# UBC-AWP/vision-sam3-yolo-lameless

Hardware: AMD Instinct MI355X
Metric: frames/sec (whole node) for YOLO+SAM3+DINOv3 feature extraction, 1080p clips (higher is better)
Workload: dtype f16; 1 GPU; BASELINE cfg#5, dense schedule: fused per-frame path on a synthetic 5 s @ 30 fps 1080p clip (150 unique BGR frames resident in HBM): YOLOv8-l detect (letterbox 384x640, NMS, scale_boxes; f16 plan) -> SAM (Hiera-B+ image encoder + FPN at 1024x1024, box-prompted mask decoder, 1080p mask + statistics + contour features) + DINOv3 ViT-L/16 embed (224x224) on EVERY frame; per-frame records packed, gathe; parallelism=one clip per GPU, 1 GPU(s), one gather per step, streams=7

## Files before the change

### vision-sam3-yolo-lameless_amd/csrc/common.h

```cpp
#pragma once
#include <hip/hip_runtime.h>
#include <stdint.h>
#include <stdio.h>
#include <stdarg.h>
#include "../../include/lmx.h"

typedef _Float16 half_t;
typedef _Float16 half2_t __attribute__((ext_vector_type(2)));
typedef _Float16 half4_t __attribute__((ext_vector_type(4)));
typedef _Float16 half8_t __attribute__((ext_vector_type(8)));
typedef float f32x4 __attribute__((ext_vector_type(4)));
typedef float f32x16 __attribute__((ext_vector_type(16)));
typedef unsigned int u32x4 __attribute__((ext_vector_type(4)));
typedef unsigned int u32x2 __attribute__((ext_vector_type(2)));

void lmx_set_error(const char* fmt, ...);

#define LMX_REQUIRE(cond, ...)            \
  do {                                    \
    if (!(cond)) {                        \
      lmx_set_error(__VA_ARGS__);         \
      return LMX_EINVAL;                  \
    }                                     \
  } while (0)

#define LMX_HIP(call)                                                                   \
  do {                                                                                  \
    hipError_t e_ = (call);                                                             \
    if (e_ != hipSuccess) {                                                             \
      lmx_set_error("%s failed: %s (%s:%d)", #call, hipGetErrorString(e_), __FILE__, __LINE__); \
      return LMX_EHIP;                                                                  \
    }                                                                                   \
  } while (0)

#define LMX_TRY(call)               \
  do {                              \
    const int rc_ = (call);         \
    if (rc_ != LMX_OK) return rc_;  \
  } while (0)

int lmx_stream_device(hipStream_t st, int* dev);
int lmx_cu_count(int dev);
int lmx_persistent_grid(int64_t need, int dev, unsigned* grid);
int lmx_allow_lds(const void* kernel, int bytes, int dev);
int lmx_env_int(const char* name, int dflt);
int lmx_env_set(const char* name);
int lmx_env_char(const char* name);

struct GemmRoute {
  bool dma;
  int BM, BN, BK, NSTAGE, STAG;
  bool rowln = false;
};
#define LMX_ROUTE_NAME(name, cap, ...)                                                                          \
  do {                                                                                                          \
    LMX_REQUIRE((name) != nullptr && (cap) > 0, "%s: no room for the name", __func__);                          \
    LMX_REQUIRE(snprintf((name), (size_t)(cap), __VA_ARGS__) < (cap), "%s: name buffer of %d bytes is too short", __func__, (cap)); \
  } while (0)

static inline int lmx_launch_check(const char* what) {
  hipError_t e = hipGetLastError();
  if (e != hipSuccess) {
    lmx_set_error("launch of %s failed: %s", what, hipGetErrorString(e));
    return LMX_EHIP;
  }
  return LMX_OK;
}

typedef float f32x2 __attribute__((ext_vector_type(2)));

__device__ __forceinline__ f32x2 gelu_pk(f32x2 v) {
  f32x2 vc;
  vc[0] = __builtin_amdgcn_fmed3f(v[0], -4.5f, 4.5f);
  vc[1] = __builtin_amdgcn_fmed3f(v[1], -4.5f, 4.5f);
  const f32x2 u = vc * vc;
  f32x2 p = {-1.223331157e-12f, -1.223331157e-12f};
  p = p * u + 1.524351007e-10f;
  p = p * u + -8.481037793e-09f;
  p = p * u + 2.798429583e-07f;
  p = p * u + -6.151207192e-06f;
  p = p * u + 9.615961466e-05f;
  p = p * u + -1.114801972e-03f;
  p = p * u + 9.814679350e-03f;
  p = p * u + -6.632144717e-02f;
  p = p * u + 3.988863025e-01f;
  const f32x2 g = vc * p;
  return v * g + 0.5f * v;
}
__device__ __forceinline__ float gelu_1(float v) {
  const f32x2 r = gelu_pk(f32x2{v, v});
  return r[0];
}

__device__ __forceinline__ float lmx_act(float v, int act) {
  if (act == LMX_ACT_SILU) return v * __builtin_amdgcn_rcpf(1.0f + __builtin_amdgcn_exp2f(-v * 1.44269504088896340736f));
  if (act == LMX_ACT_GELU) return gelu_1(v);
  if (act == LMX_ACT_RELU) return fmaxf(v, 0.0f);
  return v;
}

typedef __attribute__((address_space(3))) void* lds_ptr_t;

__device__ __forceinline__ void lds_dma16(__amdgpu_buffer_rsrc_t rs, char* dst_lds, unsigned voffset, int soffset) {
  __builtin_amdgcn_raw_ptr_buffer_load_lds(rs, (lds_ptr_t)dst_lds, 16, voffset, soffset, 0, 0);
}

#define LMX_WAIT_CASE(n) \
  if constexpr (N == n) asm volatile("s_waitcnt vmcnt(" #n ")" ::: "memory")
template <int N>
__device__ __forceinline__ void wait_vmcnt() {
  static_assert(N == 0 || N == 1 || N == 2 || N == 3 || N == 4 || N == 6 || N == 8 || N == 9 || N == 12 || N == 16 || N == 18 || N == 24 ||
                    N == 32,
                "add the literal for this count");
  LMX_WAIT_CASE(0);
  LMX_WAIT_CASE(1);
  LMX_WAIT_CASE(2);
  LMX_WAIT_CASE(3);
  LMX_WAIT_CASE(4);
  LMX_WAIT_CASE(6);
  LMX_WAIT_CASE(8);
  LMX_WAIT_CASE(9);
  LMX_WAIT_CASE(12);
  LMX_WAIT_CASE(16);
  LMX_WAIT_CASE(18);
  LMX_WAIT_CASE(24);
  LMX_WAIT_CASE(32);
}
#undef LMX_WAIT_CASE
template <int PT>
__device__ __forceinline__ void wait_tiles(int y) {
  if (y >= 4)
    wait_vmcnt<4 * PT>();
  else if (y == 3)
    wait_vmcnt<3 * PT>();
  else if (y == 2)
    wait_vmcnt<2 * PT>();
  else if (y == 1)
    wait_vmcnt<PT>();
  else
    wait_vmcnt<0>();
}

static inline bool aligned16(const void* p) { return (((uintptr_t)p) & 15) == 0; }

__device__ __forceinline__ float wave_sum(float v) {
#pragma unroll
  for (int o = 32; o > 0; o >>= 1) v += __shfl_xor(v, o, 64);
  return v;
}
__device__ __forceinline__ float wave_max(float v) {
#pragma unroll
  for (int o = 32; o > 0; o >>= 1) v = fmaxf(v, __shfl_xor(v, o, 64));
  return v;
}

__device__ __forceinline__ float act_exact(float v, int act) {
  if (act == LMX_ACT_SILU) return v / (1.0f + expf(-v));
  if (act == LMX_ACT_RELU) return fmaxf(v, 0.0f);
  if (act == LMX_ACT_GELU) return 0.5f * v * (1.0f + erff(v * 0.70710678118654752440f));
  return v;
}

__device__ __forceinline__ void bil_idx(float scale, int dst, int in_size, int& i0, int& i1, float& l1) {
  float src = scale * ((float)dst + 0.5f) - 0.5f;
  src = src < 0.f ? 0.f : src;
  i0 = (int)src;
  i1 = i0 + (i0 < in_size - 1 ? 1 : 0);
  l1 = src - (float)i0;
}

__device__ __forceinline__ float sample_mid(const float* __restrict__ lg, int L, int T, float sLT, int Y, int X) {
  int y0, y1, x0, x1;
  float ly, lx;
  bil_idx(sLT, Y, L, y0, y1, ly);
  bil_idx(sLT, X, L, x0, x1, lx);
  const float t0 = (1.f - lx) * lg[y0 * L + x0] + lx * lg[y0 * L + x1];
  const float t1 = (1.f - lx) * lg[y1 * L + x0] + lx * lg[y1 * L + x1];
  return (1.f - ly) * t0 + ly * t1;
}
```

### vision-sam3-yolo-lameless_amd/csrc/gemm.hip

```cpp
#include "common.h"
#include <stdlib.h>

namespace {

constexpr int BK = 64;

template <int BM, int BN, int AMODE, int OUT_DT>
__global__ __launch_bounds__(256, 2) void gemm_kernel(const lmx_gemm_desc p) {
  extern __shared__ __attribute__((aligned(16))) char smem[];
  half_t* As = reinterpret_cast<half_t*>(smem);
  half_t* Ws = As + 2 * BM * BK;
  constexpr int FM = BM / 32;
  constexpr int FN = BN / 32;
  constexpr int AI = BM / 32;
  constexpr int WI = BN / 32;

  const int tid = threadIdx.x;
  const int lane = tid & 63;
  const int wave = tid >> 6;
  const int wm = wave & 1, wn = wave >> 1;

  const int nwg = gridDim.x;
  const int bid = blockIdx.x;
  const int q = nwg >> 3, r = nwg & 7, xcd = bid & 7;
// ... 64 lines not shown
#pragma unroll
    for (int i = 0; i < WI; ++i)
      w_st[i] = (w_ok[i] && k_ok) ? *reinterpret_cast<const half8_t*>(W + w_off[i] + k) : zero8;
  };
  auto store_tile = [&](int buf) {
    half_t* as = As + buf * BM * BK;
    half_t* ws = Ws + buf * BN * BK;
#pragma unroll
    for (int i = 0; i < AI; ++i) {
      const int row = r0 + 32 * i;
      *reinterpret_cast<half8_t*>(as + row * BK + ((c ^ (row & 7)) << 3)) = a_st[i];
    }
#pragma unroll
    for (int i = 0; i < WI; ++i) {
      const int row = r0 + 32 * i;
      *reinterpret_cast<half8_t*>(ws + row * BK + ((c ^ (row & 7)) << 3)) = w_st[i];
    }
  };

  f32x4 acc[FM][FN];
#pragma unroll
  for (int i = 0; i < FM; ++i)
#pragma unroll
    for (int j = 0; j < FN; ++j) acc[i][j] = f32x4{0.f, 0.f, 0.f, 0.f};

  const int nk = (p.K + BK - 1) / BK;
  load_tile(0);
  store_tile(0);
  __syncthreads();

  const int frow = lane & 15;
  const int fq = lane >> 4;
  for (int kt = 0; kt < nk; ++kt) {
    const int buf = kt & 1;
    if (kt + 1 < nk) load_tile(kt + 1);
    const half_t* as = As + buf * BM * BK + (wm * (BM / 2) + frow) * BK;
    const half_t* ws = Ws + buf * BN * BK + (wn * (BN / 2) + frow) * BK;
#pragma unroll
    for (int ks = 0; ks < 2; ++ks) {
      const int coff = (((ks << 2) + fq) ^ (frow & 7)) << 3;
      half8_t af[FM], wf[FN];
#pragma unroll
      for (int i = 0; i < FM; ++i) af[i] = *reinterpret_cast<const half8_t*>(as + i * 16 * BK + coff);
#pragma unroll
      for (int j = 0; j < FN; ++j) wf[j] = *reinterpret_cast<const half8_t*>(ws + j * 16 * BK + coff);
#pragma unroll
      for (int i = 0; i < FM; ++i)
#pragma unroll
        for (int j = 0; j < FN; ++j)
          acc[i][j] = __builtin_amdgcn_mfma_f32_16x16x32_f16(wf[j], af[i], acc[i][j], 0, 0, 0);
    }
    if (kt + 1 < nk) store_tile(buf ^ 1);
    __syncthreads();
  }

  if (p.act == LMX_ACT_SWIGLU) {
    if constexpr (OUT_DT == LMX_F16 && FN % 2 == 0) {
      half_t* C = reinterpret_cast<half_t*>(p.C);
#pragma unroll
      for (int i = 0; i < FM; ++i) {
        const int m = m0 + wm * (BM / 2) + i * 16 + frow;
        if (m >= p.M) continue;
#pragma unroll
        for (int j = 0; j < FN; j += 2) {
          const int n = n0 + wn * (BN / 2) + j * 16 + fq * 4;
          if (n >= p.N) continue;
          f32x4 g = acc[i][j], u = acc[i][j + 1];
          if (p.bias) {
            g += *reinterpret_cast<const f32x4*>(p.bias + n);
            u += *reinterpret_cast<const f32x4*>(p.bias + n + 16);
          }
          const int no = (n >> 5) * 16 + (n & 15);
          f32x4 v;
#pragma unroll
          for (int e = 0; e < 4; ++e) v[e] = __fmul_rn(lmx_act(g[e], LMX_ACT_SILU), u[e]);
          if (p.scale) {
            const f32x4 s = *reinterpret_cast<const f32x4*>(p.scale + no);
#pragma unroll
            for (int e = 0; e < 4; ++e) v[e] = __fmul_rn(v[e], s[e]);
          }
          half4_t o;
#pragma unroll
          for (int e = 0; e < 4; ++e) o[e] = (half_t)v[e];
          *reinterpret_cast<half4_t*>(C + (int64_t)m * p.ldc + no) = o;
        }
      }
    }
    return;
  }

#pragma unroll
  for (int i = 0; i < FM; ++i) {
    const int m = m0 + wm * (BM / 2) + i * 16 + frow;
    if (m >= p.M) continue;
    const int mr = p.res_rows > 0 ? m % p.res_rows : m;
#pragma unroll
    for (int j = 0; j < FN; ++j) {
      const int n = n0 + wn * (BN / 2) + j * 16 + fq * 4;
      if (n >= p.N) continue;
      f32x4 v = acc[i][j];
      if (p.bias) {
        const f32x4 b = *reinterpret_cast<const f32x4*>(p.bias + n);
        v += b;
      }
      if (p.act != LMX_ACT_NONE) {
#pragma unroll
        for (int e = 0; e < 4; ++e) v[e] = lmx_act(v[e], p.act);
      }
      if (p.scale) {
        const f32x4 s = *reinterpret_cast<const f32x4*>(p.scale + n);
#pragma unroll
        for (int e = 0; e < 4; ++e) v[e] = __fmul_rn(v[e], s[e]);
      }
      if (OUT_DT == LMX_F32) {
        float* C = reinterpret_cast<float*>(p.C);
        if (p.res) {
          const f32x4 rr = *reinterpret_cast<const f32x4*>(reinterpret_cast<const float*>(p.res) + (int64_t)mr * p.ldr + n);
#pragma unroll
          for (int e = 0; e < 4; ++e) v[e] = __fadd_rn(v[e], rr[e]);
        }
        *reinterpret_cast<f32x4*>(C + (int64_t)m * p.ldc + n) = v;
      } else {
        half_t* C = reinterpret_cast<half_t*>(p.C);
        if (p.res) {
          const half4_t rr =
              *reinterpret_cast<const half4_t*>(reinterpret_cast<const half_t*>(p.res) + (int64_t)mr * p.ldr + n);
#pragma unroll
          for (int e = 0; e < 4; ++e) v[e] = __fadd_rn((float)(half_t)v[e], (float)rr[e]);
        }
        half4_t o;
#pragma unroll
        for (int e = 0; e < 4; ++e) o[e] = (half_t)v[e];
        *reinterpret_cast<half4_t*>(C + (int64_t)m * p.ldc + n) = o;
      }
    }
  }
}

template <int BM, int BN, int AMODE, int OUT_DT>
int launch(const lmx_gemm_desc& d, hipStream_t st) {
  const int MT = (d.M + BM - 1) / BM, NT = (d.N + BN - 1) / BN;
  const size_t smem = (size_t)2 * (BM + BN) * BK * sizeof(half_t);
  int dev;
  LMX_TRY(lmx_stream_device(st, &dev));
  LMX_TRY(lmx_allow_lds(reinterpret_cast<const void*>(&gemm_kernel<BM, BN, AMODE, OUT_DT>), (int)smem, dev));
  hipLaunchKernelGGL((gemm_kernel<BM, BN, AMODE, OUT_DT>), dim3(MT * NT), dim3(256), smem, st, d);
  return lmx_launch_check("gemm_kernel");
}

}

GemmRoute lmx_gemm2_tiling(const lmx_gemm_desc& d);
int lmx_gemm2_launch(const lmx_gemm_desc& d, const GemmRoute& r, hipStream_t st);

static bool dma_ok(const lmx_gemm_desc& d, int m_min, int n_min) {
  const bool a_ok = d.a_mode != 1 || (d.Cin % 32 == 0 && d.H < 32768 && d.W_ < 32768);
  return a_ok && d.M >= m_min && d.N >= n_min && d.N % 8 == 0 && d.ldc % 8 == 0 && aligned16(d.C) &&
         (!d.res || (d.ldr % 8 == 0 && aligned16(d.res)));
}

static int gemm_route(const lmx_gemm_desc* dp, GemmRoute& r) {
  LMX_REQUIRE(dp != nullptr, "lmx_k_gemm: null descriptor");
  const lmx_gemm_desc& d = *dp;
  LMX_REQUIRE(d.A && d.W && d.C, "lmx_k_gemm: null A/W/C");
  LMX_REQUIRE(d.M > 0 && d.N > 0 && d.K > 0, "lmx_k_gemm: empty problem M=%d N=%d K=%d", d.M, d.N, d.K);
  LMX_REQUIRE(d.K % 8 == 0, "lmx_k_gemm: K=%d must be a multiple of 8", d.K);
  LMX_REQUIRE(d.N % 4 == 0, "lmx_k_gemm: N=%d must be a multiple of 4", d.N);
  LMX_REQUIRE(d.lda % 8 == 0, "lmx_k_gemm: lda=%lld must be a multiple of 8", (long long)d.lda);
  const bool gated = d.act == LMX_ACT_SWIGLU;
  LMX_REQUIRE(d.ldc % 4 == 0 && d.ldc >= (gated ? d.N / 2 : d.N), "lmx_k_gemm: bad ldc=%lld", (long long)d.ldc);
  LMX_REQUIRE(aligned16(d.A) && aligned16(d.W), "lmx_k_gemm: A/W must be 16-byte aligned");
  LMX_REQUIRE((((uintptr_t)d.C) & 7) == 0, "lmx_k_gemm: C must be 8-byte aligned");
  LMX_REQUIRE(d.out_dtype == LMX_F16 || d.out_dtype == LMX_F32, "lmx_k_gemm: bad out_dtype %d", d.out_dtype);
  LMX_REQUIRE(d.out_dtype == LMX_F16 || aligned16(d.C), "lmx_k_gemm: f32 C must be 16-byte aligned");
  LMX_REQUIRE(d.act >= LMX_ACT_NONE && d.act <= LMX_ACT_SWIGLU, "lmx_k_gemm: bad act %d", d.act);
  if (gated) {
    LMX_REQUIRE(d.N % 32 == 0, "lmx_k_gemm: LMX_ACT_SWIGLU: N=%d (gate + up rows, interleaved by 16) must be a multiple of 32", d.N);
    LMX_REQUIRE(!d.res, "lmx_k_gemm: LMX_ACT_SWIGLU takes no residual");
    LMX_REQUIRE(d.a_mode == 0 && d.a_rep <= 1 && d.split_k <= 1, "lmx_k_gemm: LMX_ACT_SWIGLU: dense A only (a_mode 0; no pooled rows, convolution, a_rep or split_k); a_mode=%d", d.a_mode);
    LMX_REQUIRE(d.out_dtype == LMX_F16, "lmx_k_gemm: LMX_ACT_SWIGLU writes f16 (one rounding of the f32 product)");
  }
  if (d.bias) LMX_REQUIRE(aligned16(d.bias), "lmx_k_gemm: bias must be 16-byte aligned");
  if (d.scale) LMX_REQUIRE(aligned16(d.scale), "lmx_k_gemm: scale must be 16-byte aligned");
  if (d.res) LMX_REQUIRE(d.ldr % 4 == 0 && d.ldr >= d.N, "lmx_k_gemm: bad ldr=%lld", (long long)d.ldr);
  LMX_REQUIRE(d.res_rows >= 0, "lmx_k_gemm: res_rows");
  if (d.a_mode == 0) {
    LMX_REQUIRE(d.a_rep > 1 || d.lda >= d.K, "lmx_k_gemm: lda=%lld < K=%d", (long long)d.lda, d.K);
  } else if (d.a_mode == 1) {
    LMX_REQUIRE(d.Cin > 0 && d.Cin % 8 == 0, "lmx_k_gemm: conv Cin=%d must be a multiple of 8", d.Cin);
    LMX_REQUIRE(d.K == 9 * d.Cin, "lmx_k_gemm: conv K=%d != 9*Cin=%d", d.K, 9 * d.Cin);
    LMX_REQUIRE(d.conv_stride == 1 || d.conv_stride == 2, "lmx_k_gemm: conv stride %d", d.conv_stride);
    LMX_REQUIRE(d.H > 0 && d.W_ > 0, "lmx_k_gemm: conv H/W");
    LMX_REQUIRE(d.Ho == (d.H + 2 - 3) / d.conv_stride + 1 && d.Wo == (d.W_ + 2 - 3) / d.conv_stride + 1,
                "lmx_k_gemm: conv Ho/Wo (%d,%d) inconsistent with H/W (%d,%d) stride %d", d.Ho, d.Wo, d.H, d.W_,
                d.conv_stride);
    LMX_REQUIRE(d.M % (d.Ho * d.Wo) == 0, "lmx_k_gemm: conv M=%d not a multiple of Ho*Wo", d.M);
    LMX_REQUIRE(d.lda >= d.Cin, "lmx_k_gemm: conv pixel stride lda=%lld < Cin=%d", (long long)d.lda, d.Cin);
  } else if (d.a_mode == 2) {
    LMX_REQUIRE(d.lda >= d.K, "lmx_k_gemm: lda=%lld < K=%d", (long long)d.lda, d.K);
    LMX_REQUIRE(d.H > 0 && d.W_ > 0 && d.H % 2 == 0 && d.W_ % 2 == 0 && d.M % (d.H * d.W_) == 0,
                "lmx_k_gemm: pooled rows need an even H x W token grid that divides M (H=%d W=%d M=%d)", d.H, d.W_, d.M);
    LMX_REQUIRE(!d.res && !d.scale && d.act == LMX_ACT_NONE, "lmx_k_gemm: pooled rows: no residual / scale / activation");
    LMX_REQUIRE(((int64_t)d.M * d.lda + d.K) * 2 < 0x7fffffffll, "lmx_k_gemm: pooled rows: A must be smaller than 2 GB");
    LMX_REQUIRE(dma_ok(d, 512, 96),
                "lmx_k_gemm: pooled rows are built for the LDS-DMA kernel (M >= 512, N >= 96, N %% 8 == 0): use GEMM + maxpool2 for M=%d N=%d", d.M, d.N);
  } else {
    LMX_REQUIRE(false, "lmx_k_gemm: bad a_mode %d", d.a_mode);
  }
  LMX_REQUIRE(d.a_rep >= 0 && d.a_rep <= 3, "lmx_k_gemm: a_rep=%d (0..3)", d.a_rep);
  LMX_REQUIRE(d.split_k >= 0 && d.split_k <= 64, "lmx_k_gemm: split_k=%d (0..64)", d.split_k);
  static const int v1 = lmx_env_char("LMX_GEMM_V1") == '1';
  static const int n64 = lmx_env_char("LMX_GEMM_N64") != '0';
  if (d.ln_out) {
    LMX_REQUIRE(d.out_dtype == LMX_F32 && d.res && d.res_rows == 0, "lmx_k_gemm: ln_out needs f32 output with a full residual (out_dtype=%d res_rows=%d)", d.out_dtype, d.res_rows);
    LMX_REQUIRE(d.N <= 448 && d.N % 16 == 0 && d.K <= 448, "lmx_k_gemm: ln_out: a tile holds whole rows of N <= 448 (N %% 16 == 0) over K <= 448; N=%d K=%d", d.N, d.K);
    LMX_REQUIRE(d.a_mode == 0 && d.a_rep <= 1 && d.split_k <= 1, "lmx_k_gemm: ln_out: dense A only (a_mode=%d a_rep=%d split_k=%d)", d.a_mode, d.a_rep, d.split_k);
    LMX_REQUIRE(d.act == LMX_ACT_NONE && !d.scale, "lmx_k_gemm: ln_out takes no activation and no scale");
    LMX_REQUIRE(d.ln_gamma && d.ln_beta && aligned16(d.ln_gamma) && aligned16(d.ln_beta), "lmx_k_gemm: ln_gamma / ln_beta must be given, 16-byte aligned");
    LMX_REQUIRE(d.ld_ln % 4 == 0 && d.ld_ln >= d.N && (((uintptr_t)d.ln_out) & 7) == 0, "lmx_k_gemm: ln_out must be 8-byte aligned with ld_ln=%lld a multiple of 4, >= N", (long long)d.ld_ln);
    LMX_REQUIRE(aligned16(d.res), "lmx_k_gemm: ln_out: the residual must be 16-byte aligned");
    r = GemmRoute{true, 128, 448, BK, 2, 0, true};
    return LMX_OK;
  }
  bool dma;
  if (d.split_k > 1) {
    LMX_REQUIRE(d.out_dtype == LMX_F32 && d.act == LMX_ACT_NONE && d.a_mode != 2 && d.a_rep <= 1, "lmx_k_gemm: split_k needs f32 output, no activation, a_mode 0 or 1");
    LMX_REQUIRE(d.split_stride >= (int64_t)(d.M - 1) * d.ldc + d.N && d.split_stride % 4 == 0, "lmx_k_gemm: split_stride=%lld", (long long)d.split_stride);
    LMX_REQUIRE((d.K + 63) / 64 >= d.split_k, "lmx_k_gemm: split_k=%d exceeds the k-tiles of K=%d", d.split_k, d.K);
    LMX_REQUIRE(dma_ok(d, 1, 64),
                "lmx_k_gemm: split_k is built into the LDS-DMA kernel only (N >= 64, N %% 8 == 0; conv: Cin %% 32 == 0); M=%d N=%d", d.M, d.N);
    dma = true;
  } else if (d.a_rep > 1) {
    LMX_REQUIRE(d.a_mode == 0 && d.K % d.a_rep == 0 && (d.K / d.a_rep) % 64 == 0, "lmx_k_gemm: a_rep=%d needs a_mode 0 and K / a_rep a multiple of 64 (K=%d)", d.a_rep, d.K);
    LMX_REQUIRE(d.lda >= d.K / d.a_rep, "lmx_k_gemm: lda=%lld < K / a_rep", (long long)d.lda);
    LMX_REQUIRE(dma_ok(d, 512, 96),
                "lmx_k_gemm: a_rep is built into the LDS-DMA kernel only (M >= 512, N >= 96, N %% 8 == 0); M=%d N=%d", d.M, d.N);
    dma = true;
  } else if (d.a_mode == 2) {
    dma = true;
  } else {
    dma = !v1 && dma_ok(d, 512, d.a_mode == 1 && n64 && d.M >= 65536 ? 64 : 96);
  }
  if (dma) {
    r = lmx_gemm2_tiling(d);
  } else {
    const bool narrow = d.N <= 64 || (d.N < 128 && d.N % 128 != 0);
    r = GemmRoute{false, 128, narrow ? 64 : 128, BK, 2, 0};
  }
  return LMX_OK;
}

static constexpr int v1_key(int BN, int a_mode, int out_dtype) { return BN * 4 + a_mode * 2 + out_dtype; }

extern "C" int lmx_k_gemm(const lmx_gemm_desc* dp, lmx_stream_t stream) {
  GemmRoute r;
  LMX_TRY(gemm_route(dp, r));
  const lmx_gemm_desc& d = *dp;
  hipStream_t st = reinterpret_cast<hipStream_t>(stream);
  if (r.dma) return lmx_gemm2_launch(d, r, st);
#define LMX_V1(BN, AMODE, OUT_DT) \
  case v1_key(BN, AMODE, OUT_DT): return launch<128, BN, AMODE, OUT_DT>(d, st)
  switch (v1_key(r.BN, d.a_mode, d.out_dtype)) {
    LMX_V1(64, 0, LMX_F16);
    LMX_V1(128, 0, LMX_F16);
    LMX_V1(64, 0, LMX_F32);
    LMX_V1(128, 0, LMX_F32);
    LMX_V1(64, 1, LMX_F16);
    LMX_V1(128, 1, LMX_F16);
    LMX_V1(64, 1, LMX_F32);
    LMX_V1(128, 1, LMX_F32);
  }
#undef LMX_V1
  LMX_REQUIRE(false, "lmx_k_gemm: no register-staged kernel 128x%d for a_mode %d, out_dtype %d", r.BN, d.a_mode, d.out_dtype);
}

extern "C" int lmx_h_gemm_route(const lmx_gemm_desc* dp, char* name, int cap) {
  GemmRoute r;
  LMX_TRY(gemm_route(dp, r));
  if (r.rowln)
    LMX_ROUTE_NAME(name, cap, "dma_128xrow_ln");
  else if (r.dma)
    LMX_ROUTE_NAME(name, cap, "dma_%dx%dx%d_s%d%s", r.BM, r.BN, r.BK, r.NSTAGE, r.STAG ? "_stag" : "");
  else
    LMX_ROUTE_NAME(name, cap, "v1_%dx%d", r.BM, r.BN);
  return LMX_OK;
}
```

### vision-sam3-yolo-lameless_amd/csrc/gemm2.hip

```cpp
#include "common.h"
#include <stdlib.h>
#include <type_traits>

#ifdef LMX_DBG_TIMELINE
__device__ unsigned long long lmx_tl[8 * 16384];
extern "C" int lmx_dbg_get_timeline(void* host, int64_t bytes) { return (int)hipMemcpyFromSymbol(host, HIP_SYMBOL(lmx_tl), bytes); }
#define TL(i, v) if (threadIdx.x == 0 && swz < 16384) lmx_tl[swz * 8 + (i)] = (v)
#else
#define TL(i, v)
#endif
namespace lmx_gemm2 {

__device__ __forceinline__ float act_apply(float v, int act) { return lmx_act(v, act); }

constexpr int smem_bytes(int BM, int BN, int BK, int NSTAGE) { return NSTAGE * (BM + BN) * BK * 2 + 2 * BN * 4; }
constexpr int waves_per_simd(int BM, int BN, int BK, int NSTAGE) {
  const int smem = smem_bytes(BM, BN, BK, NSTAGE), nwave = (BM / 64) * (BN / 64);
  const int wps = (smem <= 80 * 1024 ? 2 : 1) * nwave / 4;
  return wps < 1 ? 1 : wps;
}
template <int OUT_DT, int BM, int BN, int BK, int NSTAGE, int AMODE, int STAG, bool GATED = false>
__global__ __launch_bounds__(waves_per_simd(BM, BN, BK, NSTAGE) * 256) void gemm2_kernel(const lmx_gemm_desc p, const int ntiles, const int nt_ok) {
  constexpr int NWAVE = (BM / 64) * (BN / 64);
  constexpr int STAGE_BYTES = (BM + BN) * BK * 2;
// ... 173 lines not shown
  {
    const int y = nloc - 1 < LA - 1 ? nloc - 1 : LA - 1;
    wait_tiles<PT>(y);
  }
  __builtin_amdgcn_s_barrier();
  if (grp) __builtin_amdgcn_s_barrier();
  for (int kt = 0; kt < nloc; ++kt) {
    const char* st = smem + (kt % NSTAGE) * STAGE_BYTES;
    const half_t* as = reinterpret_cast<const half_t*>(st) + (wm * 64 + frow) * BK;
    const half_t* ws = reinterpret_cast<const half_t*>(st + BM * BK * 2) + (wn * 64 + frow) * BK;
    half8_t af[BK / 32][4], wf[BK / 32][4];
#pragma unroll
    for (int ks = 0; ks < BK / 32; ++ks) {
      const int coff = (((ks << 2) + fq) ^ fsw) << 3;
#pragma unroll
      for (int j = 0; j < 4; ++j) wf[ks][j] = *reinterpret_cast<const half8_t*>(ws + j * 16 * BK + coff);
#pragma unroll
      for (int i = 0; i < 4; ++i) af[ks][i] = *reinterpret_cast<const half8_t*>(as + i * 16 * BK + coff);
    }
    if (kt + 1 < nloc) {
      const int rest = nloc - 2 - kt;
      wait_tiles<PT>(rest < LA - 2 ? (rest < 0 ? 0 : rest) : (LA - 2 < 0 ? 0 : LA - 2));
    }
    if (kt + LA < nloc) issue(kt0 + kt + LA, (kt + LA) % NSTAGE);
    asm volatile("s_waitcnt lgkmcnt(0)" ::: "memory");
    __builtin_amdgcn_s_barrier();
    __builtin_amdgcn_s_setprio(1);
#pragma unroll
    for (int ks = 0; ks < BK / 32; ++ks)
#pragma unroll
      for (int i = 0; i < 4; ++i)
#pragma unroll
        for (int j = 0; j < 4; ++j)
          acc[i][j] = __builtin_amdgcn_mfma_f32_16x16x32_f16(wf[ks][j], af[ks][i], acc[i][j], 0, 0, 0);
    __builtin_amdgcn_s_setprio(0);
    __builtin_amdgcn_s_barrier();
  }
  if (!grp) __builtin_amdgcn_s_barrier();
  }

  if (AMODE == 1 && tid < BN && n0 + tid < p.N) {
    if (p.bias && sp_ == 0) bias_v = p.bias[n0 + tid];
    if (p.scale) scale_v = p.scale[n0 + tid];
  }
  if (tid < BN) {
    bl[tid] = bias_v;
    bl[BN + tid] = scale_v;
  }
  asm volatile("s_waitcnt lgkmcnt(0)" ::: "memory");
  __builtin_amdgcn_s_barrier();
  TL(3, wall_clock64());
#ifdef LMX_DBG_NOEPI
  if (p.M > 0 && acc[0][0][0] != 12345.f) continue;
#endif
  const bool nt_out = nt_ok && OUT_DT == LMX_F16 && ((p.ldc * 2) & 127) == 0 && (int64_t)p.M * p.N >= (16ll << 20);
  char* my = smem + wave * 4608;
  auto epilogue = [&](auto act_c, auto scale_c) {
    constexpr int ACT = decltype(act_c)::value;
    constexpr bool SCALE = decltype(scale_c)::value;
    const float* blj = bl + wn * 64 + fq * 4;
    auto finish = [&](f32x4 v, int j) -> f32x4 {
      v += *reinterpret_cast<const f32x4*>(blj + j * 16);
      if constexpr (ACT == LMX_ACT_GELU) {
        const f32x2 g0 = gelu_pk(f32x2{v[0], v[1]}), g1 = gelu_pk(f32x2{v[2], v[3]});
        v = f32x4{g0[0], g0[1], g1[0], g1[1]};
      } else if constexpr (ACT != LMX_ACT_NONE) {
#pragma unroll
        for (int e = 0; e < 4; ++e) v[e] = act_apply(v[e], ACT);
      }
      if constexpr (SCALE) v *= *reinterpret_cast<const f32x4*>(blj + BN + j * 16);
      return v;
    };
    if constexpr (ACT == LMX_ACT_SWIGLU) {
      if constexpr (OUT_DT == LMX_F16 && AMODE == 0) {
        half_t* t16 = reinterpret_cast<half_t*>(my);
        constexpr int RS = 40;
        const bool nt_g = nt_ok && ((p.ldc * 2) & 127) == 0 && (int64_t)p.M * p.N >= (32ll << 20);
#pragma unroll
        for (int pass = 0; pass < 2; ++pass) {
#pragma unroll
          for (int ii = 0; ii < 2; ++ii)
#pragma unroll
            for (int jj = 0; jj < 2; ++jj) {
              const f32x4 g = acc[pass * 2 + ii][2 * jj] + *reinterpret_cast<const f32x4*>(blj + jj * 32);
              const f32x4 u = acc[pass * 2 + ii][2 * jj + 1] + *reinterpret_cast<const f32x4*>(blj + jj * 32 + 16);
              f32x4 v;
#pragma unroll
              for (int e = 0; e < 4; ++e) v[e] = __fmul_rn(act_apply(g[e], LMX_ACT_SILU), u[e]);
              if constexpr (SCALE) {
                const f32x4 sc = *reinterpret_cast<const f32x4*>(bl + BN + wn * 32 + jj * 16 + fq * 4);
#pragma unroll
                for (int e = 0; e < 4; ++e) v[e] = __fmul_rn(v[e], sc[e]);
              }
              const half4_t o = {(half_t)v[0], (half_t)v[1], (half_t)v[2], (half_t)v[3]};
              *reinterpret_cast<half4_t*>(t16 + (ii * 16 + frow) * RS + jj * 16 + fq * 4) = o;
            }
#pragma unroll
          for (int it = 0; it < 2; ++it) {
            const int row = it * 16 + (lane >> 2), c8 = lane & 3;
            const half8_t o = *reinterpret_cast<const half8_t*>(t16 + row * RS + c8 * 8);
            const int m = m0 + wm * 64 + pass * 32 + row;
            const int no = ((n0 + wn * 64) >> 1) + c8 * 8;
            if (m < p.M && no < (p.N >> 1)) {
              half8_t* dst = reinterpret_cast<half8_t*>(reinterpret_cast<half_t*>(p.C) + (int64_t)m * p.ldc + no);
              if (nt_g)
                asm volatile("global_store_dwordx4 %0, %1, off nt" ::"v"(dst), "v"(o) : "memory");
              else
                *dst = o;
            }
          }
        }
      }
    } else if constexpr (OUT_DT == LMX_F16 && AMODE == 2) {
#pragma unroll
      for (int pass = 0; pass < 4; ++pass)
#pragma unroll
        for (int j = 0; j < 4; ++j) {
          f32x4 v = finish(acc[pass][j], j);
#pragma unroll
          for (int e = 0; e < 4; ++e) {
            v[e] = fmaxf(v[e], __shfl_xor(v[e], 1, 64));
            v[e] = fmaxf(v[e], __shfl_xor(v[e], 2, 64));
          }
          const int m = m0 + wm * 64 + pass * 16 + frow;
          const int n = n0 + wn * 64 + j * 16 + fq * 4;
          if ((frow & 3) == 0 && m < p.M && n < p.N)
            *reinterpret_cast<half4_t*>(reinterpret_cast<half_t*>(p.C) + (int64_t)(m >> 2) * p.ldc + n) =
                half4_t{(half_t)v[0], (half_t)v[1], (half_t)v[2], (half_t)v[3]};
          __builtin_amdgcn_sched_barrier(0);
        }
    } else if constexpr (OUT_DT == LMX_F16) {
      half_t* t16 = reinterpret_cast<half_t*>(my);
      constexpr int RS = 72;
#pragma unroll
      for (int pass = 0; pass < 2; ++pass) {
#pragma unroll
        for (int ii = 0; ii < 2; ++ii)
#pragma unroll
          for (int j = 0; j < 4; ++j) {
            const f32x4 v = finish(acc[pass * 2 + ii][j], j);
            const half4_t o = {(half_t)v[0], (half_t)v[1], (half_t)v[2], (half_t)v[3]};
            *reinterpret_cast<half4_t*>(t16 + (ii * 16 + frow) * RS + j * 16 + fq * 4) = o;
          }
#pragma unroll
        for (int it = 0; it < 4; ++it) {
          const int row = it * 8 + (lane >> 3), c8 = lane & 7;
          half8_t o = *reinterpret_cast<const half8_t*>(t16 + row * RS + c8 * 8);
          const int m = m0 + wm * 64 + pass * 32 + row;
          const int n = n0 + wn * 64 + c8 * 8;
          if (m < p.M && n < p.N) {
            if (p.res) {
              const int mr = p.res_rows > 0 ? m % p.res_rows : m;
              const half8_t rr = *reinterpret_cast<const half8_t*>(reinterpret_cast<const half_t*>(p.res) + (int64_t)mr * p.ldr + n);
#pragma unroll
              for (int e = 0; e < 8; ++e) o[e] = (half_t)((float)o[e] + (float)rr[e]);
            }
            half8_t* dst = reinterpret_cast<half8_t*>(reinterpret_cast<half_t*>(p.C) + (int64_t)m * p.ldc + n);
            if (nt_out)
              asm volatile("global_store_dwordx4 %0, %1, off nt" ::"v"(dst), "v"(o) : "memory");
            else
              *dst = o;
          }
        }
      }
    } else if constexpr (AMODE == 2) {
#pragma unroll
      for (int pass = 0; pass < 4; ++pass)
#pragma unroll
        for (int j = 0; j < 4; ++j) {
          f32x4 v = finish(acc[pass][j], j);
#pragma unroll
          for (int e = 0; e < 4; ++e) {
            v[e] = fmaxf(v[e], __shfl_xor(v[e], 1, 64));
            v[e] = fmaxf(v[e], __shfl_xor(v[e], 2, 64));
          }
          const int m = m0 + wm * 64 + pass * 16 + frow;
          const int n = n0 + wn * 64 + j * 16 + fq * 4;
          if ((frow & 3) == 0 && m < p.M && n < p.N) *reinterpret_cast<f32x4*>(reinterpret_cast<float*>(p.C) + (int64_t)(m >> 2) * p.ldc + n) = v;
          __builtin_amdgcn_sched_barrier(0);
        }
    } else {
      float* t32 = reinterpret_cast<float*>(my);
      constexpr int RS = 68;
      const int lrow = lane >> 4, c16 = lane & 15;
      const int n = n0 + wn * 64 + c16 * 4;
      const bool has_res = p.res != nullptr && sp_ == 0;
      float* Cs = reinterpret_cast<float*>(p.C) + (int64_t)sp_ * p.split_stride;
      f32x4 rr[4];
      auto load_res = [&](int pass) {
        f32x4* d = rr;
#pragma unroll
        for (int it = 0; it < 4; ++it) {
          const int m = m0 + wm * 64 + pass * 16 + it * 4 + lrow;
          d[it] = f32x4{0.f, 0.f, 0.f, 0.f};
          if (has_res && m < p.M && n < p.N) {
            const int mr = p.res_rows > 0 ? m % p.res_rows : m;
            d[it] = *reinterpret_cast<const f32x4*>(reinterpret_cast<const float*>(p.res) + (int64_t)mr * p.ldr + n);
          }
        }
      };
#pragma unroll
      for (int pass = 0; pass < 4; ++pass) {
        load_res(pass);
#pragma unroll
        for (int j = 0; j < 4; ++j) *reinterpret_cast<f32x4*>(t32 + frow * RS + j * 16 + fq * 4) = finish(acc[pass][j], j);
#pragma unroll
        for (int it = 0; it < 4; ++it) {
          const int row = it * 4 + lrow;
          f32x4 o = *reinterpret_cast<const f32x4*>(t32 + row * RS + c16 * 4);
          const int m = m0 + wm * 64 + pass * 16 + row;
          if (m < p.M && n < p.N) {
            if (has_res) o += rr[it];
            *reinterpret_cast<f32x4*>(Cs + (int64_t)m * p.ldc + n) = o;
          }
        }
      }
    }
  };
  {
    using T = std::true_type;
    using F = std::false_type;
    const int act = p.act;
    if constexpr (GATED) {
      if (p.scale) epilogue(std::integral_constant<int, LMX_ACT_SWIGLU>{}, T{});
      else epilogue(std::integral_constant<int, LMX_ACT_SWIGLU>{}, F{});
    } else if (p.scale) {
      if (act == LMX_ACT_NONE) epilogue(std::integral_constant<int, LMX_ACT_NONE>{}, T{});
      else if (act == LMX_ACT_SILU) epilogue(std::integral_constant<int, LMX_ACT_SILU>{}, T{});
      else if (act == LMX_ACT_GELU) epilogue(std::integral_constant<int, LMX_ACT_GELU>{}, T{});
      else epilogue(std::integral_constant<int, LMX_ACT_RELU>{}, T{});
    } else {
      if (act == LMX_ACT_NONE) epilogue(std::integral_constant<int, LMX_ACT_NONE>{}, F{});
      else if (act == LMX_ACT_SILU) epilogue(std::integral_constant<int, LMX_ACT_SILU>{}, F{});
      else if (act == LMX_ACT_GELU) epilogue(std::integral_constant<int, LMX_ACT_GELU>{}, F{});
      else epilogue(std::integral_constant<int, LMX_ACT_RELU>{}, F{});
    }
  }
  __builtin_amdgcn_s_barrier();
  TL(4, wall_clock64());
  }
}

template <int BM, int BN, int BK, int NSTAGE, int AMODE, int STAG = 0>
int launch2(const lmx_gemm_desc& d, hipStream_t st) {
  const int MT = (d.M + BM - 1) / BM, NT = (d.N + BN - 1) / BN;
  const size_t smem = smem_bytes(BM, BN, BK, NSTAGE);
  int dev;
  LMX_TRY(lmx_stream_device(st, &dev));
  LMX_TRY(lmx_allow_lds(reinterpret_cast<const void*>(&gemm2_kernel<LMX_F16, BM, BN, BK, NSTAGE, AMODE, STAG>), (int)smem, dev));
  LMX_TRY(lmx_allow_lds(reinterpret_cast<const void*>(&gemm2_kernel<LMX_F32, BM, BN, BK, NSTAGE, AMODE, STAG>), (int)smem, dev));
  const int ntiles = MT * NT * (d.split_k > 1 ? d.split_k : 1);
  int grid = ntiles;
  static const int persist = lmx_env_int("LMX_GEMM2_PERSIST", 0);
  static const int nt_ok = !lmx_env_set("LMX_GEMM2_NO_NT");
  if (persist > 0 && grid > 256 * persist) grid = 256 * persist;
  if (d.act == LMX_ACT_SWIGLU) {
    if constexpr (AMODE == 0) {
      LMX_TRY(lmx_allow_lds(reinterpret_cast<const void*>(&gemm2_kernel<LMX_F16, BM, BN, BK, NSTAGE, AMODE, STAG, true>), (int)smem, dev));
      hipLaunchKernelGGL((gemm2_kernel<LMX_F16, BM, BN, BK, NSTAGE, AMODE, STAG, true>), dim3(grid), dim3(BM * BN / 64), smem, st, d, ntiles, nt_ok);
      return lmx_launch_check("gemm2_kernel (gated)");
    } else {
      return LMX_EINVAL;
    }
  }
  if (d.out_dtype == LMX_F16)
    hipLaunchKernelGGL((gemm2_kernel<LMX_F16, BM, BN, BK, NSTAGE, AMODE, STAG>), dim3(grid), dim3(BM * BN / 64), smem, st, d, ntiles, nt_ok);
  else
    hipLaunchKernelGGL((gemm2_kernel<LMX_F32, BM, BN, BK, NSTAGE, AMODE, STAG>), dim3(grid), dim3(BM * BN / 64), smem, st, d, ntiles, nt_ok);
  return lmx_launch_check("gemm2_kernel");
}

constexpr int RL_BM = 128, RL_BN = 448, RL_BK = 64, RL_NSTAGE = 2;
constexpr int RL_STAGE_BYTES = (RL_BM + RL_BN) * RL_BK * 2;
constexpr int RL_RS = RL_BN + 4;
constexpr int RL_SMEM = RL_NSTAGE * RL_STAGE_BYTES + 3 * RL_BN * 4;
static_assert(2 * 32 * RL_RS * 4 <= RL_NSTAGE * RL_STAGE_BYTES, "two 32-row epilogue buffers inside the ring");

__device__ __forceinline__ void wave_sum4(float (&v)[4]) {
#pragma unroll
  for (int o = 32; o > 0; o >>= 1) {
    float t[4];
#pragma unroll
    for (int r = 0; r < 4; ++r) t[r] = __shfl_xor(v[r], o, 64);
#pragma unroll
    for (int r = 0; r < 4; ++r) v[r] += t[r];
  }
}

__global__ __launch_bounds__(512) void gemm2_rowln_kernel(const lmx_gemm_desc p) {
  constexpr int BM = RL_BM, BN = RL_BN, BK = RL_BK, NSTAGE = RL_NSTAGE, STAGE_BYTES = RL_STAGE_BYTES;
  constexpr int NWAVE = 8;
  constexpr int A_INSTR = BM * BK * 2 / 1024 / NWAVE;
  constexpr int W_INSTR = BN * BK * 2 / 1024 / NWAVE;
  constexpr int FJ = BN / 4 / 16;
  extern __shared__ __attribute__((aligned(16))) char smem[];
  const int tid = threadIdx.x;
  const int lane = tid & 63;
  const int wave = __builtin_amdgcn_readfirstlane(tid >> 6);
  const int wm = wave & 1, wn = wave >> 1;
  const int swz = blockIdx.x;
  const int m0 = swz * BM;
  TL(0, (unsigned long long)__builtin_amdgcn_s_getreg((31 << 11) | 4));
  TL(1, (unsigned long long)__builtin_amdgcn_s_getreg((31 << 11) | 20));
  TL(2, wall_clock64());
  TL(5, (unsigned long long)swz);

  const char* Ab = reinterpret_cast<const char*>(p.A) + (int64_t)m0 * p.lda * 2;
  int64_t a_bytes = ((int64_t)(p.M - m0 - 1) * p.lda + p.K) * 2;
// ... 243 lines not shown
```

Before: 819.9 frames/s.

## Add halo-tiled 3x3 conv kernel for 64-channel stride-1 convolutions

Adds a dedicated persistent kernel for 3x3 stride-1 convolutions with 64 input and 64 output channels. It loads each 16x16 output tile's 18x18 input halo into LDS once and reuses it across all nine taps, instead of the implicit-GEMM path re-gathering im2col rows. All weights stay resident in LDS, halos are double-buffered with async buffer-to-LDS DMA, and the bias, SiLU and residual epilogue is fused into the kernel. The path is on by default and can be switched off with LMX_CONV_HALO=0. It only covers C64 convolutions, likely the YOLO/FPN blocks, so the gain is limited to those layers, and the new kernel risks lower occupancy from its large LDS footprint.

```diff
diff --git a/vision-sam3-yolo-lameless_amd/csrc/common.h b/vision-sam3-yolo-lameless_amd/csrc/common.h
--- a/vision-sam3-yolo-lameless_amd/csrc/common.h
+++ b/vision-sam3-yolo-lameless_amd/csrc/common.h
@@ -51,6 +51,7 @@
   bool dma;
   int BM, BN, BK, NSTAGE, STAG;
   bool rowln = false;
+  bool halo = false;
 };
 #define LMX_ROUTE_NAME(name, cap, ...)                                                                          \
   do {                                                                                                          \
@@ -97,6 +98,12 @@
   if (act == LMX_ACT_GELU) return gelu_1(v);
   if (act == LMX_ACT_RELU) return fmaxf(v, 0.0f);
   return v;
+}
+
+__device__ __forceinline__ half8_t lmx_add_res_f16(half8_t o, half8_t rr) {
+#pragma unroll
+  for (int e = 0; e < 8; ++e) o[e] = (half_t)((float)o[e] + (float)rr[e]);
+  return o;
 }
 
 typedef __attribute__((address_space(3))) void* lds_ptr_t;
diff --git a/vision-sam3-yolo-lameless_amd/csrc/conv.hip b/vision-sam3-yolo-lameless_amd/csrc/conv.hip
--- /dev/null
+++ b/vision-sam3-yolo-lameless_amd/csrc/conv.hip
@@ -0,0 +1,206 @@
+#include "common.h"
+#include <type_traits>
+
+namespace lmx_conv {
+
+constexpr int TILE = 16, HALO = TILE + 2, HALO_PX = HALO * HALO;
+constexpr int PIECES = (HALO_PX + 7) / 8;
+constexpr int SLOT_BYTES = PIECES * 1024;
+constexpr int W_BYTES = 64 * 576 * 2;
+constexpr int NWAVE = 8, ROUNDS = (PIECES + NWAVE - 1) / NWAVE;
+constexpr int SMEM = W_BYTES + 2 * SLOT_BYTES + 64 * 4;
+static_assert(SMEM <= 160 * 1024, "LDS");
+
+__global__ __launch_bounds__(512) void conv_halo_c64_kernel(const lmx_gemm_desc p, const int ntiles, const int TY, const int TX) {
+  extern __shared__ __attribute__((aligned(16))) char smem[];
+  const int tid = threadIdx.x;
+  const int lane = tid & 63;
+  const int wave = __builtin_amdgcn_readfirstlane(tid >> 6);
+  const unsigned OOB = 0x80000000u;
+
+  const int bid = blockIdx.x, xcd = bid & 7;
+  const int q = ntiles >> 3, r = ntiles & 7;
+  const int base = xcd < r ? xcd * (q + 1) : r * (q + 1) + (xcd - r) * q;
+  const int cnt = q + (xcd < r ? 1 : 0);
+  const int stride = ((int)gridDim.x + 7 - xcd) >> 3;
+  int li = bid >> 3;
+  if (li >= cnt) return;
+
+  const int lpx = lane >> 3;
+  const int lchunk = (lane & 7) ^ lpx;
+  int h_yx[ROUNDS];
+#pragma unroll
+  for (int j = 0; j < ROUNDS; ++j) {
+    const int px = (wave + NWAVE * j) * 8 + lpx;
+    const int hy = px / HALO, hx = px - hy * HALO;
+    h_yx[j] = px < HALO_PX ? ((hy << 8) | hx) : -1;
+  }
+  const int img_px = p.H * p.W_;
+  const int a_bytes = ((img_px - 1) * (int)p.lda + 64) * 2;
+
+  struct Tile {
+    int img, y0, x0;
+  };
+  auto tile_of = [&](int l) {
+    const int t = base + l;
+    const int img = t / (TY * TX), rem = t - img * (TY * TX);
+    const int ty = rem / TX;
+    return Tile{img, ty * TILE, (rem - ty * TX) * TILE};
+  };
+  auto issue_halo = [&](const Tile& t, int slot) {
+    const char* Ab = reinterpret_cast<const char*>(p.A) + (int64_t)t.img * img_px * p.lda * 2;
+    const __amdgpu_buffer_rsrc_t a_rs = __builtin_amdgcn_make_buffer_rsrc(const_cast<char*>(Ab), 0, a_bytes, 0x00020000);
+    char* st = smem + W_BYTES + slot * SLOT_BYTES;
+#pragma unroll
+    for (int j = 0; j < ROUNDS; ++j) {
+      const int piece = wave + NWAVE * j;
+      if (piece < PIECES) {
+        const int iy = t.y0 - 1 + (h_yx[j] >> 8), ix = t.x0 - 1 + (h_yx[j] & 0xff);
+        const bool ok = h_yx[j] >= 0 && (unsigned)iy < (unsigned)p.H && (unsigned)ix < (unsigned)p.W_;
+        lds_dma16(a_rs, st + piece * 1024, ok ? (unsigned)((iy * p.W_ + ix) * (int)p.lda * 2 + lchunk * 16) : OOB, 0);
+      }
+    }
+  };
+
+  const int frow = lane & 15, fq = lane >> 4;
+  const bool odd = fq & 1;
+  const bool pre = wave >= NWAVE / 2;
+  const int cb0 = (odd ? 16 : 0) + (fq >> 1) * 8;
+  const half_t* res = reinterpret_cast<const half_t*>(p.res);
+  half_t* C = reinterpret_cast<half_t*>(p.C);
+  const half8_t zero8 = {0, 0, 0, 0, 0, 0, 0, 0};
+  int64_t e_m[2];
+  half8_t rr[2][2];
+  auto load_res = [&](const Tile& t) {
+#pragma unroll
+    for (int i = 0; i < 2; ++i) {
+      const int oy = t.y0 + 2 * wave + i, ox = t.x0 + frow;
+      e_m[i] = (oy < p.H && ox < p.W_) ? (int64_t)t.img * img_px + oy * p.W_ + ox : -1;
+#pragma unroll
+      for (int s = 0; s < 2; ++s) {
+        rr[i][s] = zero8;
+        if (res && e_m[i] >= 0) {
+          const int64_t mr = p.res_rows > 0 ? e_m[i] % p.res_rows : e_m[i];
+          rr[i][s] = *reinterpret_cast<const half8_t*>(res + mr * p.ldr + cb0 + 32 * s);
+        }
+      }
+    }
+  };
+
+  {
+    const __amdgpu_buffer_rsrc_t w_rs = __builtin_amdgcn_make_buffer_rsrc(const_cast<void*>(p.W), 0, W_BYTES, 0x00020000);
+#pragma unroll
+    for (int j = 0; j < 9; ++j) {
+      const int piece = wave * 9 + j, tap = piece >> 3, n = (piece & 7) * 8 + lpx;
+      lds_dma16(w_rs, smem + piece * 1024, (unsigned)(n * 1152 + tap * 128 + lchunk * 16), 0);
+    }
+  }
+  float* bl = reinterpret_cast<float*>(smem + W_BYTES + 2 * SLOT_BYTES);
+  if (tid < 64) bl[tid] = p.bias ? p.bias[tid] : 0.f;
+  Tile cur = tile_of(li);
+  issue_halo(cur, 0);
+  if (li + stride < cnt) issue_halo(tile_of(li + stride), 1);
+  load_res(cur);
+  wait_vmcnt<0>();
+  asm volatile("s_waitcnt lgkmcnt(0)" ::: "memory");
+  __builtin_amdgcn_s_barrier();
+
+  for (int it_ = 0; li < cnt; li += stride, ++it_) {
+    const int slot = it_ & 1;
+    const char* hs = smem + W_BYTES + slot * SLOT_BYTES;
+    f32x4 acc[2][4];
+#pragma unroll
+    for (int i = 0; i < 2; ++i)
+#pragma unroll
+      for (int j = 0; j < 4; ++j) acc[i][j] = f32x4{0.f, 0.f, 0.f, 0.f};
+    const int px0 = 2 * wave * HALO + frow;
+    const char* wrow = smem + frow * 128;
+    const int wsw = frow & 7;
+    half8_t af[2][2], wf[2][4];
+    auto read_frags = [&](int kc, int b) __attribute__((always_inline)) {
+      const int tap = kc >> 1, c = (kc & 1) * 4 + fq;
+      const int ky = tap / 3, kx = tap - 3 * ky;
+      const int pa = px0 + ky * HALO + kx, pb = pa + HALO;
+#pragma unroll
+      for (int j = 0; j < 4; ++j) wf[b][j] = *reinterpret_cast<const half8_t*>(wrow + tap * 8192 + j * 2048 + ((c ^ wsw) << 4));
+      af[b][0] = *reinterpret_cast<const half8_t*>(hs + pa * 128 + ((c ^ (pa & 7)) << 4));
+      af[b][1] = *reinterpret_cast<const half8_t*>(hs + pb * 128 + ((c ^ (pb & 7)) << 4));
+    };
+    read_frags(0, 0);
+#pragma unroll
+    for (int kc = 0; kc < 18; ++kc) {
+      if (kc + 1 < 18) read_frags(kc + 1, (kc + 1) & 1);
+      __builtin_amdgcn_s_setprio(1);
+#pragma unroll
+      for (int i = 0; i < 2; ++i)
+#pragma unroll
+        for (int j = 0; j < 4; ++j)
+          acc[i][j] = __builtin_amdgcn_mfma_f32_16x16x32_f16(wf[kc & 1][j], af[kc & 1][i], acc[i][j], 0, 0, 0);
+      __builtin_amdgcn_s_setprio(0);
+    }
+
+    wait_vmcnt<0>();
+
+    auto epilogue = [&](auto act_c) __attribute__((always_inline)) {
+      constexpr int ACT = decltype(act_c)::value;
+#pragma unroll
+      for (int i = 0; i < 2; ++i) {
+        half4_t o[4];
+#pragma unroll
+        for (int j = 0; j < 4; ++j) {
+          f32x4 v = acc[i][j] + *reinterpret_cast<const f32x4*>(bl + j * 16 + fq * 4);
+          if constexpr (ACT != LMX_ACT_NONE) {
+#pragma unroll
+            for (int e = 0; e < 4; ++e) v[e] = lmx_act(v[e], ACT);
+          }
+          o[j] = half4_t{(half_t)v[0], (half_t)v[1], (half_t)v[2], (half_t)v[3]};
+        }
+#pragma unroll
+        for (int s = 0; s < 2; ++s) {
+          typedef int int2_t __attribute__((ext_vector_type(2)));
+          const int2_t give = __builtin_bit_cast(int2_t, odd ? o[2 * s] : o[2 * s + 1]);
+          const int2_t got = {__shfl_xor(give[0], 16, 64), __shfl_xor(give[1], 16, 64)};
+          const half4_t mine = odd ? o[2 * s + 1] : o[2 * s], theirs = __builtin_bit_cast(half4_t, got);
+          const half4_t lo = odd ? theirs : mine, hi = odd ? mine : theirs;
+          half8_t out = {lo[0], lo[1], lo[2], lo[3], hi[0], hi[1], hi[2], hi[3]};
+          if (e_m[i] >= 0) {
+            if (res) out = lmx_add_res_f16(out, rr[i][s]);
+            *reinterpret_cast<half8_t*>(C + e_m[i] * p.ldc + cb0 + 32 * s) = out;
+          }
+        }
+      }
+    };
+    auto run_epilogue = [&]() __attribute__((always_inline)) {
+      if (p.act == LMX_ACT_SILU)
+        epilogue(std::integral_constant<int, LMX_ACT_SILU>{});
+      else
+        epilogue(std::integral_constant<int, LMX_ACT_NONE>{});
+    };
+    if (pre) run_epilogue();
+    asm volatile("s_waitcnt lgkmcnt(0)" ::: "memory");
+    __builtin_amdgcn_s_barrier();
+    const bool more = li + stride < cnt;
+    if (li + 2 * stride < cnt) issue_halo(tile_of(li + 2 * stride), slot);
+    if (!pre) run_epilogue();
+    if (more) {
+      cur = tile_of(li + stride);
+      load_res(cur);
+    }
+  }
+}
+
+}
+
+int lmx_conv_halo_launch(const lmx_gemm_desc& d, hipStream_t st) {
+  using namespace lmx_conv;
+  const int TY = (d.H + TILE - 1) / TILE, TX = (d.W_ + TILE - 1) / TILE;
+  const int64_t ntiles = (int64_t)(d.M / (d.H * d.W_)) * TY * TX;
+  LMX_REQUIRE(ntiles < 0x7fffffffll, "lmx_k_gemm: %lld halo tiles", (long long)ntiles);
+  int dev;
+  LMX_TRY(lmx_stream_device(st, &dev));
+  LMX_TRY(lmx_allow_lds(reinterpret_cast<const void*>(&conv_halo_c64_kernel), SMEM, dev));
+  unsigned grid;
+  LMX_TRY(lmx_persistent_grid(ntiles, dev, &grid));
+  hipLaunchKernelGGL(conv_halo_c64_kernel, dim3(grid), dim3(NWAVE * 64), SMEM, st, d, (int)ntiles, TY, TX);
+  return lmx_launch_check("conv_halo_c64_kernel");
+}
diff --git a/vision-sam3-yolo-lameless_amd/csrc/gemm.hip b/vision-sam3-yolo-lameless_amd/csrc/gemm.hip
--- a/vision-sam3-yolo-lameless_amd/csrc/gemm.hip
+++ b/vision-sam3-yolo-lameless_amd/csrc/gemm.hip
@@ -240,6 +240,7 @@
 
 GemmRoute lmx_gemm2_tiling(const lmx_gemm_desc& d);
 int lmx_gemm2_launch(const lmx_gemm_desc& d, const GemmRoute& r, hipStream_t st);
+int lmx_conv_halo_launch(const lmx_gemm_desc& d, hipStream_t st);
 
 static bool dma_ok(const lmx_gemm_desc& d, int m_min, int n_min) {
   const bool a_ok = d.a_mode != 1 || (d.Cin % 32 == 0 && d.H < 32768 && d.W_ < 32768);
@@ -310,6 +311,13 @@
     r = GemmRoute{true, 128, 448, BK, 2, 0, true};
     return LMX_OK;
   }
+  static const int halo = lmx_env_char("LMX_CONV_HALO") != '0';
+  if (halo && !v1 && d.a_mode == 1 && d.conv_stride == 1 && d.Cin == 64 && d.N == 64 && d.out_dtype == LMX_F16 && !d.scale &&
+      d.split_k <= 1 && d.a_rep <= 1 && (d.act == LMX_ACT_NONE || d.act == LMX_ACT_SILU) && dma_ok(d, 1, 64) &&
+      (int64_t)d.H * d.W_ * d.lda * 2 < 0x7fffffffll) {
+    r = GemmRoute{true, 256, 64, 64, 2, 0, false, true};
+    return LMX_OK;
+  }
   bool dma;
   if (d.split_k > 1) {
     LMX_REQUIRE(d.out_dtype == LMX_F32 && d.act == LMX_ACT_NONE && d.a_mode != 2 && d.a_rep <= 1, "lmx_k_gemm: split_k needs f32 output, no activation, a_mode 0 or 1");
@@ -345,6 +353,7 @@
   LMX_TRY(gemm_route(dp, r));
   const lmx_gemm_desc& d = *dp;
   hipStream_t st = reinterpret_cast<hipStream_t>(stream);
+  if (r.halo) return lmx_conv_halo_launch(d, st);
   if (r.dma) return lmx_gemm2_launch(d, r, st);
 #define LMX_V1(BN, AMODE, OUT_DT) \
   case v1_key(BN, AMODE, OUT_DT): return launch<128, BN, AMODE, OUT_DT>(d, st)
@@ -367,6 +376,8 @@
   LMX_TRY(gemm_route(dp, r));
   if (r.rowln)
     LMX_ROUTE_NAME(name, cap, "dma_128xrow_ln");
+  else if (r.halo)
+    LMX_ROUTE_NAME(name, cap, "halo_16x16_c64");
   else if (r.dma)
     LMX_ROUTE_NAME(name, cap, "dma_%dx%dx%d_s%d%s", r.BM, r.BN, r.BK, r.NSTAGE, r.STAG ? "_stag" : "");
   else
diff --git a/vision-sam3-yolo-lameless_amd/csrc/gemm2.hip b/vision-sam3-yolo-lameless_amd/csrc/gemm2.hip
--- a/vision-sam3-yolo-lameless_amd/csrc/gemm2.hip
+++ b/vision-sam3-yolo-lameless_amd/csrc/gemm2.hip
@@ -349,8 +349,7 @@
             if (p.res) {
               const int mr = p.res_rows > 0 ? m % p.res_rows : m;
               const half8_t rr = *reinterpret_cast<const half8_t*>(reinterpret_cast<const half_t*>(p.res) + (int64_t)mr * p.ldr + n);
-#pragma unroll
-              for (int e = 0; e < 8; ++e) o[e] = (half_t)((float)o[e] + (float)rr[e]);
+              o = lmx_add_res_f16(o, rr);
             }
             half8_t* dst = reinterpret_cast<half8_t*>(reinterpret_cast<half_t*>(p.C) + (int64_t)m * p.ldc + n);
             if (nt_out)
```

Measured after the change: 823.0 frames/s (median of 4 runs). Within noise of the previous version (+0.4%).
